# OpenResearchInstitute/ka9q-sdr

Measured on AMD Instinct MI355X. Metric: input Msamples/s + channels @ real-time, 16384-pt overlap-save, higher is better.
Workload: dtype f32

## Files before the change

### ka9q_sdr_amd/csrc/kq_bank.cpp

```cpp
#include <cstdarg>

#include "kq_bank.hpp"

using namespace kq::bank;

namespace {
thread_local std::string g_err;

int ilog2(unsigned v) {
  int l = 0;
  while ((1u << l) < v) l++;
  return l;
}
}

void kq_internal_set_error(const char *fmt, ...) {
  char buf[512];
  va_list ap;
  va_start(ap, fmt);
  vsnprintf(buf, sizeof buf, fmt, ap);
  va_end(ap);
  g_err = buf;
}

// ... 153 lines not shown
    b->fwd_mode = KQ_FWD_PRUNED;
  } else if (cfg->fwd_mode == KQ_FWD_FULL) {
    b->fwd_mode = KQ_FWD_FULL;
  } else {
    b->fwd_mode = (can_prune && g.Ndec != 256) ? KQ_FWD_PRUNED : KQ_FWD_FULL;
  }
  b->use64k = b->fwd_mode == KQ_FWD_FULL && can64k;
  if (b->fwd_mode == KQ_FWD_FULL && N > 16384 && !b->use64k && (!kq::split_supported(g) || cfg->compute_n0)) {
    kq_internal_set_error("N = %u: the full path beyond 16384 points needs N = 65536, or compute_n0 off and a split N = S x N1 with N1 <= 16384 a "
                          "size of its own (N = 32768; 19200, 24000, 38400, 48000 ...) and N/D small enough to sit beside it in LDS", N);
    return -1;
  }
  return 0;
}

static int create_alloc(kq_bank *b) {
  const kq_bank_config *cfg = &b->cfg;
  kq::Geom const &g = b->g;
  if (b->open_stream(cfg->stream)) return -1;
  size_t const C = cfg->max_channels, B = cfg->max_blocks;
  b->ring_cap = (size_t)(g.M - 1) + B * (size_t)g.L + (size_t)(g.L - 1);
  if (b->alloc(&b->ring[0], b->ring_cap, true)) return -1;
  if (b->alloc(&b->ring[1], b->ring_cap, true)) return -1;
  if (!(b->tw = kq::half_twiddles(g.tw_log2))) {
    kq_internal_set_error("kq_bank_create: no twiddle table of period 2^%d", g.tw_log2);
    return -1;
  }
  if (b->alloc(&b->chd.mode, C, true)) return -1;
  if (b->alloc(&b->chd.flags, C, true)) return -1;
  if (b->alloc(&b->chd.low, C, true)) return -1;
  if (b->alloc(&b->chd.high, C, true)) return -1;
  if (b->alloc(&b->chd.resp, C * g.Ndec, true)) return -1;
  if (b->alloc(&b->chd.aresp, C * (g.Ndec / 2 + 1), true)) return -1;
  if (b->alloc(&b->chd.fm_gain, C, true)) return -1;
  if (b->alloc(&b->chd.headroom, C, true)) return -1;
  if (b->alloc(&b->chd.recovery, C, true)) return -1;
  if (b->alloc(&b->chd.hangmax, C, true)) return -1;
  if (b->alloc(&b->chd.noise_gain, C, true)) return -1;
  if (b->alloc(&b->chd.hist_len, C, true)) return -1;
  if (b->alloc(&b->chd.hist2_len, C * kq::kOldLevels, true)) return -1;
  if (b->alloc(&b->chd.hist2_osc, 3 * C * kq::kOldLevels, true)) return -1;
  if (b->cfg.compute_n0 && (kq::full16k_supported(g) || b->use64k)) {
    size_t const nsub = b->use64k ? 4 : 1;
    if (b->alloc(&b->chd.n0lane, C * nsub * 256, true)) return -1;
    if (b->alloc(&b->chd.n0meta, C * nsub, true)) return -1;
    if (b->alloc(&b->chd.n0slot, C, true)) return -1;
  }
  if (b->use64k) {
    if (b->alloc(&b->big.sync, C * cfg->max_blocks * 12, true)) return -1;
    if (b->alloc(&b->big.n0part, C * cfg->max_blocks * 4, true)) return -1;
    if (b->alloc(&b->big.xs, C * cfg->max_blocks * (size_t)g.Ndec, true)) return -1;
    if (b->alloc_pinned(&b->big.err, 1)) return -1;
    *b->big.err = 0;
  }
  for (int k = 0; k < 2; k++)
    if (b->alloc(&b->osc_dev2[k], 8 * C + (B + sizeof(double) - 1) / sizeof(double) + (C * sizeof(int) + 7) / 8, true)) return -1;
  const char *ov = getenv("KQ_DEMOD_OVERLAP");
  b->overlap_mode = ov ? (atoi(ov) != 0 ? 1 : 0) : -1;
  bool const overlap = b->overlap_mode != 0;
  if (!overlap) b->stream2 = b->stream;
  if (overlap && b->new_stream(&b->stream2)) return -1;
  for (hipEvent_t &e : b->ev_demod_done)
    if (b->new_event(&e, hipEventDisableTiming)) return -1;
  b->stage_bytes = 8 * C * sizeof(double) + ((B + 7) & ~(size_t)7) + ((C * sizeof(int) + 7) & ~(size_t)7);
  b->patch_off = b->stage_bytes;
  b->stage_bytes += (size_t)kq_bank::kMaxPatch * kq_bank::kPatchBytes;
  b->bits_off = b->stage_bytes;
  b->stage_bytes += ((C + 63) / 64) * sizeof(unsigned long long);
  static_assert(kq_bank::kSlots == 4, "slot_bit_words");
  for (int k = 0; k < kq_bank::kSlots; k++) {
    if (b->alloc_pinned(&b->stage_host[k], b->stage_bytes) || b->new_event(&b->stage_ev[k], hipEventDefault) ||
        b->new_event(&b->stage_t0[k], hipEventDefault))
      return -1;
    memset(b->stage_host[k] + b->bits_off, 0, b->stage_bytes - b->bits_off);
  }
  if (b->alloc(&b->chd.fm_state, C, true)) return -1;
  if (b->alloc(&b->chd.lastaudio, C, true)) return -1;
  if (b->alloc(&b->chd.sq_count, C, true)) return -1;
  if (b->alloc(&b->chd.ahist, C * (size_t)(g.Mdec > 1 ? g.Mdec - 1 : 1), true)) return -1;
  if (!kq::demod64_supported(g)) {
    if (b->alloc(&b->fmout, C * B * (size_t)g.olen, true)) return -1;
    for (float *&h : b->fm_hist)
      if (b->alloc(&h, C * (size_t)(g.Mdec > 1 ? g.Mdec - 1 : 1), true)) return -1;
  }
  if (b->alloc(&b->chd.foffset, C, true)) return -1;
  if (b->alloc(&b->chd.pdev, C, true)) return -1;
  if (b->alloc(&b->chd.gain, C, true)) return -1;
  if (b->alloc(&b->chd.hang, C, true)) return -1;
  if (b->alloc(&b->chd.dc, C, true)) return -1;
  if (b->alloc(&b->chd.n0, C, true)) return -1;
  if (b->alloc(&b->chd.pl_ptr, C, true)) return -1;
  if (b->alloc(&b->chd.pl_last, C, true)) return -1;
  if (b->alloc(&b->chd.plfreq, C, true)) return -1;
  if (g.pl_n > 0) {
    if (b->alloc(&b->chd.plresp, (size_t)g.pl_n / 2 + 1, true)) return -1;
    if (b->alloc(&b->chd.plring, C * 16384, true)) return -1;
  }
  if (b->alloc(&b->pl.audio, C * B * 2 * (size_t)g.olen, true)) return -1;
  if (b->alloc(&b->pl.status, C * B, true)) return -1;
  for (int k = 0; k < 2; k++) {
    b->pl2[k].audio = b->pl.audio;
    b->pl2[k].status = b->pl.status;
    if (b->alloc(&b->pl2[k].filt, C * B * g.olen, true)) return -1;
    if (b->alloc(&b->pl2[k].n0raw, C * B, true)) return -1;
    if (b->alloc(&b->pl2[k].if_power, B * (1 + kq::kEnergySplitMax), true)) return -1;
    if (g.pl_n > 0 && b->alloc(&b->pl2[k].plout, C * B * g.pl_l, true)) return -1;
// ... 141 lines not shown
```

### ka9q_sdr_amd/csrc/kq_bank_call.cpp

```cpp
#include "kq_bank.hpp"

using namespace kq::bank;

namespace kq::bank {

void harvest_slot(kq_bank *b, int slot) {
  if (!b->stage_timed[slot]) return;
  b->stage_timed[slot] = false;
  float ms = 0;
  if (hipEventElapsedTime(&ms, b->stage_t0[slot], b->stage_ev[slot]) == hipSuccess && ms > 0) {
    b->acc.filter_ms += ms;
    if (ms > b->acc.filter_max_ms) {
      b->acc.filter_max_ms = ms;
      b->acc.filter_max_submit_ms = b->stage_submit_ms[slot];
      b->acc.filter_max_launch = b->stage_launch[slot];
    }
  } else
    (void)hipGetLastError();
}

void note_retune(kq_bank *b, int ch) {
  HostChan &h = b->chans[ch];
  int64_t const hist = (int64_t)b->g.M - 1;
  if (h.retuned && h.hist_old == hist) return;
// ... 330 lines not shown
      for (unsigned i = 0; i < k.nblocks; i++) {
        const float2 *X = k.spectrum + (size_t)i * g.N;
        size_t const cb = (size_t)c * g.max_blocks + i;
        if (b->cfg.compute_n0)
          kq::launch_n0_single(b->stream, X, g.N, g.samprate, b->chans[c].cfg.low, b->chans[c].cfg.high, k.pl.n0raw + cb);
        kq::launch_slave_bank(b->stream, X, k.chd.resp + (size_t)c * g.Ndec, k.pl.filt + cb * g.olen, g.N, g.Ndec, g.olen, isb ? 2 : 1,
                              b->tw, g.tw_log2);
      }
    }
  } else if (b->fwd_mode == KQ_FWD_PRUNED) {
    if (b->chan_tw_dirty) {
      kq::launch_pruned_tables(b->stream, g, k.chd, b->chan_tw, k.C);
      b->chan_tw_dirty = false;
    }
    if (kq::pruned_carries_iir(g)) iir_arm(b, k);
    kq::launch_filter_pruned(b->stream, g, k.chd, k.pl, k.window, b->chan_tw, act.n, nblocks, k.swept_pruned, act.list, b->big.iir);
    b->big.iir = kq::IirArgs{};
    if (k.nret > 0) {
      if (g.N > 16384)
        kq::launch_filter_split(b->stream, g, k.chd, k.pl, k.window, b->tw, k.nret, (int)k.nredo, k.retune_list);
      else
        full_launch(b, k, k.nret, (int)k.nredo, k.retune_list, 0, false);
    }
  } else if (b->use64k) {
    launch64k(b, k, act.n, nblocks, act.list, k.plain);
    if (k.plain && k.nret > 0) launch64k(b, k, k.nret, (int)k.nredo, k.retune_list, false);
  } else if (g.N > 16384) {
    kq::launch_filter_split(b->stream, g, k.chd, k.pl, k.window, b->tw, k.C, nblocks, nullptr);
  } else {
    int const steady_variant = k.swept_steady ? 2 : k.plain ? 1 : 0;
    if (k.mixed) {
      full_launch(b, k, (int)b->list_unswept_host.size(), nblocks, b->list_unswept_dev, 1);
      full_launch(b, k, (int)b->list_swept_host.size(), nblocks, b->list_swept_dev, steady_variant);
    } else {
      full_launch(b, k, act.n, nblocks, act.list, steady_variant);
    }
    if (k.use16k && (k.plain || k.mixed || k.swept_steady) && k.nret > 0)
      full_launch(b, k, k.nret, (int)k.nredo, k.retune_list, 0);
  }
}

int launch_energy_and_filter(kq_bank *b, Call &k) {
  kq::Geom const &g = b->g;
  int const slot = k.slot, pp = k.pp;
  if (ctl_flush(b, CTL_FILTER, b->stream)) return -1;
  {
    Scope t(b, 2, b->stream);
    kq::launch_block_energy_sum(b->stream, k.spectrum ? nullptr : k.window + (g.M - 1), g.L, k.spectrum ? 0 : (int)k.nblocks,
                                k.pl.if_power + b->cfg.max_blocks,
                                b->stage_host[slot], b->osc_dev2[pp],
                                k.nret ? k.ret_off + k.nret * sizeof(int) : 8 * k.Cmax * sizeof(double) + k.nblocks,
                                k.spectrum ? nullptr : k.paired, (int)(g.M - 1), k.steady ? b->osc_dev2[pp ^ 1] : nullptr, (unsigned)k.C,
                                (unsigned)k.Cmax, (double)(k.n_w - b->planes_n_w), (double)(b->out_abs - b->planes_out_abs),
                                b->stage_host[slot] + b->patch_off, k.npatch, b->stage_host[slot] + b->bits_off);
  }
  LAUNCH_CHECK("IF power");
  if (b->timing) {
    KQ_TRY(hipEventRecord(b->stage_t0[slot], b->stream));
    b->stage_timed[slot] = true;
    b->stage_h0[slot] = std::chrono::steady_clock::now();
    b->stage_launch[slot] = b->acc.filter_launches;
  }
  static bool const iir_in_filter_off = getenv("KQ_IIR_IN_FILTER") && atoi(getenv("KQ_IIR_IN_FILTER")) == 0;
  k.iir_off = iir_in_filter_off;
  launch_filter(b, k);
  LAUNCH_CHECK("pre-detection filter");
  b->acc.filter_launches++;
  b->acc.channel_blocks += (uint64_t)k.C * k.nblocks;
  KQ_TRY(hipEventRecord(b->stage_ev[slot], b->stream));
  if (b->timing) b->stage_submit_ms[slot] = std::chrono::duration<double, std::milli>(std::chrono::steady_clock::now() - b->stage_h0[slot]).count();
  return 0;
}

int launch_demodulators(kq_bank *b, Call &k) {
  kq::Geom const &g = b->g;
  int const pp = k.pp, nblocks = (int)k.nblocks;
  kq::Planes const &pl = k.pl;
  kq::ChanDev const &chd = k.chd;
  bool const agc_channels = !b->list_host[1].empty() || !b->list_host[2].empty();
  bool const overlap = b->stream2 != b->stream &&
                       (b->overlap_mode == 1 || (b->overlap_mode < 0 && !b->use64k && (b->pulled_since_call || agc_channels)));
  b->pulled_since_call = false;
  hipStream_t const ds = overlap ? b->stream2 : b->stream;
  int const prev = pp ^ 1;
  if (overlap)
    KQ_TRY(hipStreamWaitEvent(ds, b->stage_ev[k.slot], 0));
  else if (b->calls > 0 && b->demod_overlapped[prev])
    KQ_TRY(hipStreamWaitEvent(ds, b->ev_demod_done[prev], 0));
  if (b->out_pending) {
    KQ_TRY(hipStreamWaitEvent(ds, b->pull_done[(b->pulls - 1) % kq_bank::kPullRing], 0));
    b->out_pending = false;
  }
  if (ctl_flush(b, CTL_DEMOD, ds)) return -1;
  if (k.spectrum)
    KQ_TRY(hipMemsetAsync(pl.if_power, 0, k.nblocks * sizeof(float), ds));
  else if (!k.iir_done)
    kq::launch_block_energy_iir(ds, pl.if_power + b->cfg.max_blocks, g.L, nblocks,
                                reinterpret_cast<const unsigned char *>(b->osc_dev2[pp] + 8 * k.Cmax), b->energy_state, pl.if_power);
  {
    Scope t(b, 1, ds);
    int const nfm = (int)b->list_host[0].size(), nam = (int)b->list_host[1].size(), nlin = (int)b->list_host[2].size();
    bool const fused_fm = kq::demod64_supported(g);
    kq::launch_demod64(ds, g, chd, pl, b->list_dev[0], fused_fm ? nfm : 0, b->list_dev[1], nam, b->list_dev[2], nlin, nblocks,
                       b->cfg.compute_n0);
    if (!fused_fm) {
      kq::launch_demod_fm(ds, g, chd, pl, b->tw, b->list_dev[0], nfm, nblocks, b->cfg.compute_n0, b->fmout,
                          b->fm_hist[b->fm_hist_cur], b->fm_hist[b->fm_hist_cur ^ 1]);
// ... 166 lines not shown
```

### ka9q_sdr_amd/csrc/kq_device.hpp

```cpp
#pragma once
#include "kq_energy.hpp"
#include <hip/hip_runtime.h>
#include <stdint.h>

#include <functional>

#include "../../include/ka9q_hip.h"

struct filter_in;

namespace kq {

enum { FLAG_FLAT = 1, FLAG_ISB = 2, FLAG_STEREO = 4, FLAG_SQUARE = 8 };

struct PllState {
  double c_phase, c_freq;
  double f_phase, f_freq;
  float integrator, delta_f, snr, foffset, cphase;
  int lock_count, pll_lock, fft_samples, fft_ptr;
};

struct FftDim {
  int n;
  int log2n;
  int nf;
  unsigned char f[12];
  const unsigned short *rev;
  const float2 *twc;
  int tw_n;
};
FftDim fft_dim(int n, bool *ok);
bool fft_size_ok(int n);
const float2 *half_twiddles(int log2T);
enum { TABLE_HALF_TWIDDLES, TABLE_DIM_REV, TABLE_DIM_TW, TABLE_FULL16K };
const void *upload_once(int table, int size, size_t bytes, const std::function<void(void *)> &fill);

constexpr int kPllChunk = 64;
struct PllChunk {
  PllState *state;
  float2 *rings;
  float2 *side;
};

struct Geom {
  int N, L, M, D;
  FftDim dN, dNdec, dPl;
  int Ndec, olen, Mdec;
  int log2N, log2Ndec;
  int samprate;
  int tw_log2;
  int max_blocks;
  float dsamprate;
  int pl_n, pl_l;
};

constexpr int kOldLevels = 4;

struct ChanDev {
  int *mode;
  int *flags;
  int *fflags;
  float *low, *high;
  float2 *resp;
  float2 *aresp;
  float *fm_gain;
  float *headroom;
  float *recovery;
  int *hangmax;
  float *noise_gain;
  unsigned long long *n0lane;
  unsigned *n0meta;
  int *n0slot;
  double *lo_phase, *lo_freq, *lo_rate;
  double *hist_phase, *hist_freq, *hist_rate;
  int *hist_len;
  int *hist2_len;
  double *hist2_osc;
  double *sh_phase, *sh_freq;
  float2 *fm_state;
  float *lastaudio;
  int *sq_count;
  float *ahist;
  float *foffset, *pdev;
  float *gain;
  int *hang;
  float *dc;
  float *n0;
  float2 *plresp;
  float *plring;
  int *pl_ptr, *pl_last;
  float *plfreq;
};

struct Planes {
  float2 *filt;
  float *audio;
  kq_chan_status *status;
  float *n0raw;
  float *if_power;
  float *plout;
};

struct DeviceScope {
  int prev = -1;
  bool switched = false;
  explicit DeviceScope(int device) {
    if (device < 0) return;
    if (hipGetDevice(&prev) == hipSuccess && prev != device) switched = hipSetDevice(device) == hipSuccess;
  }
  ~DeviceScope() {
    if (switched) (void)hipSetDevice(prev);
  }
  DeviceScope(const DeviceScope &) = delete;
  DeviceScope &operator=(const DeviceScope &) = delete;
};

void ensure_dynamic_lds(const void *kernel, size_t bytes);

void launch_copy_to_host(hipStream_t s, const float *audio, float *haudio, int row, const kq_chan_status *status, void *hstatus,
                         size_t rows);
void launch_copy_pcm_to_host(hipStream_t s, const float *audio, short *hpcm, unsigned *hmask, int row,
                             const kq_chan_status *status, void *hstatus, size_t rows, const int *mode_compact = nullptr,
                             int max_blocks = 1);
void launch_ingest(hipStream_t s, const void *src, int format, float2 *dst, size_t nsamples, float scale);
constexpr int kEnergySplitMax = 16;
int block_energy_split(int L);
void launch_block_energy_sum(hipStream_t s, const float2 *newsamples, int L, int nblocks, float *sums, const void *params_host,
                             void *params_dev, size_t params_bytes, float2 *paired, int hist, const double *prev_planes = nullptr,
                             unsigned nchan = 0, unsigned cmax = 0, double adv = 0, double adv_out = 0, const void *patch_records_host = nullptr,
                             int npatch = 0, const void *patch_bits_host = nullptr);
void launch_ctl_apply(hipStream_t s, const void *queue_host, int nrec);
void launch_block_energy_iir(hipStream_t s, const float *sums, int L, int nblocks, const unsigned char *update, float *energy_state,
                             float *if_power);
void launch_pcm(hipStream_t s, const Geom &g, const Planes &pl, short *pcm, unsigned *mask, int nchan, int nblocks,
                const int *chan_list);
void launch_filter_full(hipStream_t s, const Geom &g, const ChanDev &ch, const Planes &pl, const float2 *window,
                        const float2 *tw, int nchan, int nblocks, int compute_n0, float2 *spec_dump, int spec_ch,
                        const int *chan_list);
bool split_supported(const Geom &g);
void launch_filter_split(hipStream_t s, const Geom &g, const ChanDev &ch, const Planes &pl, const float2 *window,
                         const float2 *tw, int nchan, int nblocks, const int *chan_list);
struct Big64 {
  unsigned long long *sync;
  float2 *n0part;
  float2 *xs;
  int *err;
  unsigned epoch;
  IirArgs iir;
};
bool full16k_supported(const Geom &g);
constexpr int kFull16kHalf = 16;
constexpr int full16k_bin(int t) { return (t >> 5) + 32 * (t & 31); }
void launch_filter_full16k(hipStream_t s, const Geom &g, const ChanDev &ch, const Planes &pl, const float2 *window,
                           const float2 *tw, int nchan, int nblocks, int compute_n0, float2 *spec_dump, int spec_ch,
                           const int *chan_list, int plain, const float2 *window_paired, const Big64 &big);
bool full16k_paired_supported(const Geom &g);
bool full64k_supported(const Geom &g);
void launch_filter_full64k(hipStream_t s, const Geom &g, const ChanDev &ch, const Planes &pl, const float2 *window,
                           const float2 *tw, int nchan, int nblocks, int compute_n0, float2 *spec_dump, int spec_ch,
                           const int *chan_list, bool plain, bool swept, const float2 *window_paired, const Big64 &big);
double full16k_sweep_limit();
double full64k_sweep_limit();
bool pruned_supported(const Geom &g);
void launch_filter_pruned(hipStream_t s, const Geom &g, const ChanDev &ch, const Planes &pl, const float2 *window,
                          const float2 *chan_tw, int nchan, int nblocks, bool swept, const int *chan_list, const IirArgs &iir = IirArgs{});
bool pruned_carries_iir(const Geom &g);
void launch_pruned_tables(hipStream_t s, const Geom &g, const ChanDev &ch, float2 *chan_tw, int nchan);
size_t pruned_table_elems(const Geom &g);
size_t demod_fm_lds_bytes(const Geom &g);
void launch_demod_fm(hipStream_t s, const Geom &g, const ChanDev &ch, const Planes &pl, const float2 *tw, const int *list_fm,
                     int n_fm, int nblocks, int compute_n0, float *fmout, const float *fm_hist_in, float *fm_hist_out);
void launch_pl_track(hipStream_t s, const Geom &g, const ChanDev &ch, const Planes &pl, const float2 *tw, const int *list_fm,
                     int n_fm, int nblocks);
bool demod64_supported(const Geom &g);
void launch_demod64(hipStream_t s, const Geom &g, const ChanDev &ch, const Planes &pl, const int *list_fm, int n_fm,
                    const int *list_am, int n_am, const int *list_lin, int n_lin, int nblocks, int compute_n0);
void launch_demod_pll(hipStream_t s, const Geom &g, const ChanDev &ch, const Planes &pl, const float2 *tw, const int *list_pll,
                      int n_pll, const PllChunk *chunks, const int *slot_of, int nblocks, int compute_n0);
void launch_fft_single(hipStream_t s, const float2 *in, float2 *out, const FftDim &d, int sign, const float2 *tw, int tw_log2);
int launch_fft_large(hipStream_t s, const float2 *in, float2 *out, float2 *tmp, int N, int sign, const float2 *tw, int tw_log2);
void launch_n0_single(hipStream_t s, const float2 *fdomain, int N, int samprate, float low, float high, float *out);
void launch_slave_single(hipStream_t s, const float2 *fdomain, const float2 *resp, float2 *out, int N, int Ndec,
                         int in_real, int out_type, const float2 *tw, int tw_log2);
// ... 10 lines not shown
```

### ka9q_sdr_amd/csrc/kq_full16k.hip

```cpp
#include "kq_device.hpp"
#include "kq_ldsfft.hpp"
#include <cmath>
#include <type_traits>

#include "kq_lane.hpp"
#include "kq_regfft.hpp"

#ifdef KQ_TIMELINE
__device__ unsigned long long kq_timeline[64][8][12];
#define KQ_STAMP(i)                                                                        \
  do {                                                                                     \
    __builtin_amdgcn_sched_barrier(0);                                                     \
    if (blockIdx.y == (gridDim.y > 40 ? 40 : gridDim.y / 2) && (blockIdx.x & 15) == 0 && (blockIdx.x >> 4) < 64 &&      \
        (threadIdx.x & 63) == 0)                                                           \
      kq_timeline[blockIdx.x >> 4][threadIdx.x >> 6][i] = clock64();                       \
    __builtin_amdgcn_sched_barrier(0);                                                     \
  } while (0)
extern "C" int kq_debug_timeline(unsigned long long *dst) {
  return hipMemcpyFromSymbol(dst, HIP_SYMBOL(kq_timeline), sizeof(kq_timeline)) == hipSuccess ? 0 : -1;
}
#else
#define KQ_STAMP(i)
#endif

// ... 76 lines not shown
    for (;;) {
      w = __hip_atomic_load(slots + t, __ATOMIC_RELAXED, __HIP_MEMORY_SCOPE_AGENT);
      if ((unsigned)(w >> 32) == tag || ++it > (1 << 18)) break;
      __builtin_amdgcn_s_sleep(8);
    }
    if ((unsigned)(w >> 32) != tag) {
      *err = 1;
      w = 0x7fc00000u;
    }
    out[t] = __uint_as_float((unsigned)w);
  }
  __syncthreads();
}

}

template <bool N0, bool DUMP, int PLAIN, bool PAIRED, int BIG, int EPI>
__global__ __launch_bounds__(kT, 4) void k_filter_full16k(Geom g, ChanDev ch, Planes pl, const float2 *__restrict__ window,
                                                       const float2 *__restrict__ tw, const float2 *__restrict__ tab,
                                                       float2 *__restrict__ spec_dump, int spec_ch,
                                                       const int *__restrict__ chan_list, Big64 big) {
  extern __shared__ __attribute__((aligned(16))) float2 xch[];
  __shared__ __attribute__((aligned(16))) float2 stab[(kT / 64) * (BIG ? 128 : 32)];
  __shared__ float sib_f[BIG ? 12 : 1];
  constexpr int kNfull = BIG ? 4 * kN : kN;
  int const r4 = BIG ? (int)(blockIdx.x & 3) : 0;
  __shared__ __attribute__((aligned(16))) float2 tw2[16 * kTw2Pitch];
  __shared__ float red_f[2][kT / 64];
  __shared__ float red_c[kT / 64];
  __shared__ int red_i[2][kT / 64];
  int const t = threadIdx.x;
  int const Ndec = g.Ndec;
  KQ_STAMP(0);
  __builtin_amdgcn_s_setprio(3);
  v2f v[32];
  rsrc_t const xr = make_rsrc(window + (size_t)blockIdx.y * g.L, kNfull * (unsigned)sizeof(float2));
  unsigned const toff = (unsigned)t * (unsigned)sizeof(float2);
  auto load_rows = [&](int first, int last) {
    if constexpr (PAIRED) {
#pragma unroll
      for (int n1 = first; n1 < last; n1 += 2)
        buf_ld4(v[rfft::bitrev5(n1)], v[rfft::bitrev5(n1 + 1)], xr, 2 * toff, (unsigned)(n1 / 2) * (unsigned)(1024 * sizeof(float2)));
    } else {
#pragma unroll
      for (int n1 = first; n1 < last; n1++) v[rfft::bitrev5(n1)] = buf_ld2(xr, toff, (unsigned)n1 * (unsigned)(512 * sizeof(float2)));
    }
  };
  auto load_window = [&]() { load_rows(0, 32); };
  rsrc_t const tabr = make_rsrc(tab, kTabSize * (unsigned)sizeof(float2));
  v2f tlo[3], thi[7];
  int const cidx = BIG ? (int)(blockIdx.x >> 2) : (int)blockIdx.x;
  int const c = chan_list ? chan_list[cidx] : cidx, b = blockIdx.y;
  v2f pt = (v2f){1.f, 0.f};
  if constexpr (BIG != 0) {
    double const ph0 = ch.lo_phase[c], f0 = ch.lo_freq[c], rs = ch.lo_rate[c];
    double const hp0 = ch.hist_phase[c], hf0 = ch.hist_freq[c], hr = ch.hist_rate[c];
    double const mbase = (double)b * g.L;
    int const n_old = (hp0 != ph0 || hf0 != f0 || hr != rs) ? ch.hist_len[c] - b * g.L : 0;
    bool const retuned = n_old > 0;
    if (PLAIN || (!retuned && fabs(rs) <= kSweepLimit64k)) {
      constexpr bool kSwept = !PLAIN || BIG == 2;
      v2f sa[2][4], sb[2][4];
      auto issue = [&](int i, int slot) {
#pragma unroll
        for (int j = 0; j < 4; j++) {
          if constexpr (PAIRED) {
            buf_ld4(sa[slot][j], sb[slot][j], xr, 2 * toff, (unsigned)(16 * j + i) * (unsigned)(1024 * sizeof(float2)));
          } else {
            sa[slot][j] = buf_ld2(xr, toff, (unsigned)(32 * j + 2 * i) * (unsigned)(512 * sizeof(float2)));
            sb[slot][j] = buf_ld2(xr, toff, (unsigned)(32 * j + 2 * i + 1) * (unsigned)(512 * sizeof(float2)));
          }
        }
      };
      issue(0, 0);
      issue(1, 1);
      __builtin_amdgcn_sched_barrier(0);
      float2 *const sw = stab + (t >> 6) * 128;
      {
        int const lane = t & 63;
        double const wv = (double)(64 * (t >> 6));
#pragma unroll
        for (int e2 = 0; e2 < 2; e2++) {
          int const e = lane + 64 * e2, j = e >> 5, n1 = e & 31;
          double const R = (double)(16384 * j + 512 * n1), U = mbase + R;
          double turns = f0 * U - (double)(r4 * n1) * (1.0 / 128.0) - 0.25 * (double)(r4 * j);
          if (kSwept) turns += rs * (0.5 * U * (U - 1.0) + R * wv);
          sw[e] = phasor_turns(turns);
        }
      }
      {
        double const td = (double)t;
        double turns = ph0 + f0 * td - (double)(r4 * t) * (1.0 / 65536.0);
        if (kSwept) turns += rs * (mbase * td + 0.5 * td * (td - 1.0));
        pt = phasor2(turns);
      }
      float const kbf = kSwept ? (float)(2.0 * M_PI * 16384.0 * rs * (double)(t & 63)) : 0.f;
      v2f const kb = (v2f){kbf, kbf};
      __builtin_amdgcn_fence(__ATOMIC_RELEASE, "wavefront");
      __builtin_amdgcn_wave_barrier();
      __builtin_amdgcn_fence(__ATOMIC_ACQUIRE, "wavefront");
      const float4 *const tp = reinterpret_cast<const float4 *>(sw);
#pragma unroll
      for (int i = 0; i < 16; i++) {
        int const slot = i & 1;
        float4 tt[4];
#pragma unroll
        for (int j = 0; j < 4; j++) tt[j] = tp[16 * j + i];
#pragma unroll
        for (int e = 0; e < 2; e++) {
          int const n1 = 2 * i + e;
          v2f x[4], w[4];
#pragma unroll
          for (int j = 0; j < 4; j++) {
            x[j] = e ? sb[slot][j] : sa[slot][j];
            w[j] = e ? (v2f){tt[j].z, tt[j].w} : (v2f){tt[j].x, tt[j].y};
          }
          v2f z;
          if constexpr (kSwept) {
            v2f const y0 = pk_cmul(x[0], w[0]), y1 = pk_cmul(x[1], w[1]), y2 = pk_cmul(x[2], w[2]), y3 = pk_cmul(x[3], w[3]);
            v2f const a = y1 + y3, bb = y2 + y3;
            v2f const S = (y0 + y2) + a;
            v2f const W = rfft::pk_fma(bb, (v2f){2.f, 2.f}, a);
            v2f const Uu = n1 ? rfft::pk_fma(S, (v2f){n1 / 32.f, n1 / 32.f}, W) : W;
            asm("v_pk_fma_f32 %0, %1, %2, %3 op_sel:[1,0,0] op_sel_hi:[0,1,1] neg_lo:[0,1,0]" : "=v"(z) : "v"(Uu), "v"(kb), "v"(S));
          } else {
            z = pk_cmul(x[0], w[0]);
            z = rfft::pk_cmadd(x[1], w[1], z);
            z = rfft::pk_cmadd(x[2], w[2], z);
            z = rfft::pk_cmadd(x[3], w[3], z);
          }
          v[rfft::bitrev5(n1)] = z;
        }
        if (i + 2 < 16) issue(i + 2, slot);
      }
    } else {
      OlderOsc older;
      load_older(ch, c, b * g.L, n_old > 0, older);
#pragma unroll
      for (int n1 = 0; n1 < 32; n1++) {
        v2f acc = (v2f){0.f, 0.f};
        for (int j = 0; j < 4; j++) {
          int const i = 16384 * j + 512 * n1 + t;
          double const m = mbase + i;
          bool const old = i < n_old;
          double pp = old ? hp0 : ph0, ff = old ? hf0 : f0, rr = old ? hr : rs;
          pick_older(older, i, pp, ff, rr);
          double turns = pp + ff * m;
          if (rr != 0.0) turns += rr * (0.5 * m * (m - 1.0));
          turns -= (double)(r4 * (512 * n1 + t)) * (1.0 / 65536.0) + 0.25 * (double)(r4 * j);
          acc = rfft::pk_cmadd(buf_ld2(xr, toff, (unsigned)(32 * j + n1) * (unsigned)(512 * sizeof(float2))), phasor2(turns), acc);
        }
        v[rfft::bitrev5(n1)] = acc;
      }
    }
  }
  if constexpr (PLAIN && BIG == 0) {
    double const ph0 = ch.lo_phase[c], f0 = ch.lo_freq[c];
    double const rs = PLAIN == 2 ? ch.lo_rate[c] : 0.0;
    load_rows(0, 12);
    __builtin_amdgcn_sched_barrier(0);
    float2 *const sw = stab + (t >> 6) * 32;
    if ((t & 63) < 32) {
      double const R = (double)(512 * (t & 63));
      double turns = f0 * R;
      if constexpr (PLAIN == 2) turns += rs * (0.5 * R * (R - 1.0) + R * ((double)b * g.L + (double)(t & ~63)));
      sw[t & 63] = phasor_turns(turns);
    }
    __builtin_amdgcn_sched_barrier(0);
    load_rows(12, 22);
    __builtin_amdgcn_sched_barrier(0);
    {
      double const A = (double)b * g.L + t;
      double turns = ph0 + f0 * A;
      if constexpr (PLAIN == 2) turns += rs * (0.5 * A * (A - 1.0));
      pt = phasor2(turns);
    }
    __builtin_amdgcn_sched_barrier(0);
    load_rows(22, 32);
  }
  twiddle32_fetch(tlo, thi, tabr, t);
  v2f const tw2_mine = buf_ld2(tabr, toff, (unsigned)kTabTw2 * 8u);
  KQ_STAMP(10);

  if constexpr (BIG == 0) {
    double const ph0 = ch.lo_phase[c], f0 = ch.lo_freq[c], r = ch.lo_rate[c];
    double const hp0 = ch.hist_phase[c], hf0 = ch.hist_freq[c], hr = ch.hist_rate[c];
    double const mbase = (double)b * g.L;
    int const n_old = (hp0 != ph0 || hf0 != f0 || hr != r) ? ch.hist_len[c] - b * g.L : 0;
    bool const retuned = n_old > 0;
    if (PLAIN || (r == 0.0 && !retuned)) {
      float2 *const sw = stab + (t >> 6) * 32;
      if constexpr (!PLAIN) {
        load_window();
        if ((t & 63) < 32) sw[t & 63] = phasor_turns(f0 * (double)(512 * (t & 63)));
        pt = phasor2(ph0 + f0 * (mbase + t));
      }
      KQ_STAMP(11);
      __builtin_amdgcn_fence(__ATOMIC_RELEASE, "wavefront");
      __builtin_amdgcn_wave_barrier();
      __builtin_amdgcn_fence(__ATOMIC_ACQUIRE, "wavefront");
      if constexpr (PLAIN == 2) {
        float const kbf = (float)(2.0 * M_PI * 512.0 * r * (double)(t & 63));
        v2f const kb = (v2f){kbf, kbf};
        v2f th = (v2f){0.f, 0.f};
#pragma unroll
        for (int n1 = 1; n1 < 32; n1++) {
          v2f const y = pk_cmul(v[rfft::bitrev5(n1)], ld2(sw + n1));
          th = th + kb;
          v2f z;
          asm("v_pk_fma_f32 %0, %1, %2, %3 op_sel:[1,0,0] op_sel_hi:[0,1,1] neg_lo:[0,1,0]" : "=v"(z) : "v"(y), "v"(th), "v"(y));
          v[rfft::bitrev5(n1)] = z;
        }
      } else {
#pragma unroll
        for (int n1 = 1; n1 < 32; n1++) v[rfft::bitrev5(n1)] = pk_cmul(v[rfft::bitrev5(n1)], ld2(sw + n1));
      }
    } else if constexpr (!PLAIN) {
      OlderOsc older;
      load_older(ch, c, b * g.L, n_old > 0, older);
#pragma unroll
      for (int n1 = 0; n1 < 32; n1++) {
        int const i = 512 * n1 + t;
        double const m = mbase + i;
        bool const old = i < n_old;
        double pp = old ? hp0 : ph0, ff = old ? hf0 : f0, rr = old ? hr : r;
        pick_older(older, i, pp, ff, rr);
        double turns = pp + ff * m;
        if (rr != 0.0) turns += rr * (0.5 * m * (m - 1.0));
        v[rfft::bitrev5(n1)] = pk_cmul(buf_ld2(xr, toff, (unsigned)n1 * (unsigned)(512 * sizeof(float2))), phasor2(turns));
      }
    }
  }

  KQ_STAMP(1);
  __builtin_amdgcn_s_setprio(0);
  rfft::fft_dit_pk<32>(v);
  twiddle32(v, tlo, thi, pt);

  KQ_STAMP(2);
  v2f u[32];
  tw2[(t >> 5) * kTw2Pitch + (t & 31)] = make_float2(tw2_mine.x, tw2_mine.y);
#if defined(KQ_ABLATE) && (KQ_ABLATE & 1)
#pragma unroll
  for (int n2 = 0; n2 < 32; n2++) u[n2] = v[n2];
#else
  {
    int const rd = ((t >> 4) & 15) * kRow1 + (t & 15);
#pragma unroll
// ... 420 lines not shown
      G[bitrev((unsigned)k, g.log2Ndec)] = gn;
    }
    G[bitrev((unsigned)p, g.log2Ndec)] = gp;
  }
  lds_fft<+1>(G, g.log2Ndec, tw, g.tw_log2);
  float2 *o = pl.filt + cb * g.olen;
  for (int i = t; i < g.olen; i += blockDim.x) o[i] = G[Ndec - g.olen + i];
}

bool full16k_supported(const Geom &g) {
  return g.N == kN && 2 * g.Ndec <= kXchElems && g.Ndec >= 4;
}

static const float2 *twiddle_tables() {
  return (const float2 *)upload_once(TABLE_FULL16K, kN, kTabSize * sizeof(float2), [](void *bytes) {
    float2 *h = (float2 *)bytes;
    auto w = [](long long e) {
      double const ang = -2.0 * M_PI * (double)(e % kN) / kN;
      return make_float2((float)cos(ang), (float)sin(ang));
    };
    for (int t = 0; t < kT; t++)
      for (int e = 0; e < 10; e++)
        h[kTabP1 + 2 * (kT * (e >> 1) + t) + (e & 1)] = e < 3 ? w((long long)(e + 1) * t) : w(4LL * (e - 2) * t);
    for (int n3 = 0; n3 < 16; n3++)
      for (int k2 = 0; k2 < 32; k2++) h[kTabTw2 + 32 * n3 + k2] = w(32LL * n3 * k2);
    for (int st = 1; st <= 5; st++)
      for (int t = 0; t < 64; t++) {
        int const half = 1 << st;
        double const ang = M_PI * (double)(t & (half - 1)) / half;
        h[kTabEpi + (st - 1) * 64 + t] = (t & half) ? make_float2((float)cos(ang), (float)sin(ang)) : make_float2(1.f, 0.f);
      }
  });
}

bool full16k_paired_supported(const Geom &g) {
  return (full16k_supported(g) || full64k_supported(g)) && g.L % 1024 == 0 && (g.M - 1) % 1024 == 0;
}

bool full64k_supported(const Geom &g) { return g.N == 4 * kN && g.Ndec >= 4 && g.Ndec <= 16384; }
double full64k_sweep_limit() { return kSweepLimit64k; }
double full16k_sweep_limit() { return kSweepLimit16k; }

void launch_filter_full16k(hipStream_t s, const Geom &g, const ChanDev &ch, const Planes &pl, const float2 *window,
                           const float2 *tw, int nchan, int nblocks, int compute_n0, float2 *spec_dump, int spec_ch,
                           const int *chan_list, int plain, const float2 *window_paired, const Big64 &big) {
  size_t const lds_bytes = (size_t)kXchElems * sizeof(float2);
  const float2 *tab = twiddle_tables();
  if (!tab) {
    launch_filter_full(s, g, ch, pl, window, tw, nchan, nblocks, compute_n0, spec_dump, spec_ch, chan_list);
    if (big.iir.sums)
      launch_block_energy_iir(s, big.iir.sums, big.iir.L, big.iir.nblocks, big.iir.update, big.iir.state, big.iir.if_power);
    return;
  }
  bool const n0 = compute_n0 && ch.n0lane && ch.n0meta;
  bool const dump = spec_dump != nullptr;
  bool const paired = plain && window_paired != nullptr;
  auto go = [&](auto kernel) {
    ensure_dynamic_lds((const void *)kernel, lds_bytes);
    hipLaunchKernelGGL(kernel, dim3(nchan, nblocks), dim3(kT), lds_bytes, s, g, ch, pl, paired ? window_paired : window, tw, tab,
                       spec_dump, spec_ch, chan_list, big);
  };
  int const epi = dump ? 0 : g.Ndec == 64 ? 1 : (g.Ndec >= 128 && g.Ndec <= 512) ? 2 : 0;
  auto pick3 = [&](auto n0c, auto dumpc, auto epic) {
    constexpr bool kN0 = decltype(n0c)::value, kDump = decltype(dumpc)::value;
    constexpr int kEpi = decltype(epic)::value;
    if (plain == 2)
      paired ? go(k_filter_full16k<kN0, kDump, 2, true, 0, kEpi>) : go(k_filter_full16k<kN0, kDump, 2, false, 0, kEpi>);
    else if (paired)
      go(k_filter_full16k<kN0, kDump, 1, true, 0, kEpi>);
    else
      plain ? go(k_filter_full16k<kN0, kDump, 1, false, 0, kEpi>) : go(k_filter_full16k<kN0, kDump, 0, false, 0, kEpi>);
  };
  auto pick = [&](auto n0c, auto dumpc) {
    if constexpr (decltype(dumpc)::value) {
      pick3(n0c, dumpc, std::integral_constant<int, 0>{});
    } else {
      if (epi == 1)
        pick3(n0c, dumpc, std::integral_constant<int, 1>{});
      else if (epi == 2)
        pick3(n0c, dumpc, std::integral_constant<int, 2>{});
      else
        pick3(n0c, dumpc, std::integral_constant<int, 0>{});
    }
  };
  using T = std::true_type;
  using F = std::false_type;
  if (n0)
    dump ? pick(T{}, T{}) : pick(T{}, F{});
  else
    dump ? pick(F{}, T{}) : pick(F{}, F{});
}

void launch_filter_full64k(hipStream_t s, const Geom &g, const ChanDev &ch, const Planes &pl, const float2 *window,
                           const float2 *tw, int nchan, int nblocks, int compute_n0, float2 *spec_dump, int spec_ch,
                           const int *chan_list, bool plain, bool swept, const float2 *window_paired, const Big64 &big) {
  size_t const lds_bytes = (size_t)kXchElems * sizeof(float2);
  const float2 *tab = twiddle_tables();
  if (!tab) {
    if (big.iir.sums)
      launch_block_energy_iir(s, big.iir.sums, big.iir.L, big.iir.nblocks, big.iir.update, big.iir.state, big.iir.if_power);
    return;
  }
  bool const n0 = compute_n0 && ch.n0lane && ch.n0meta;
  bool const dump = spec_dump != nullptr;
  bool const paired = plain && window_paired != nullptr;
  auto go = [&](auto kernel) {
// ... 27 lines not shown
```

### ka9q_sdr_amd/csrc/kq_kernels.hip

```cpp
#include <algorithm>
#include <map>
#include <mutex>
#include <utility>

#include "kq_device.hpp"
#include "kq_ctl.hpp"
#include "kq_energy.hpp"
#include "kq_ldsfft.hpp"

namespace kq {

void ensure_dynamic_lds(const void *kernel, size_t bytes) {
  static std::mutex mu;
  static std::map<std::pair<const void *, int>, size_t> limit;
  int dev = 0;
  if (hipGetDevice(&dev) != hipSuccess) return;
  std::lock_guard<std::mutex> lock(mu);
  size_t &cur = limit[{kernel, dev}];
  if (bytes > cur) {
    (void)hipFuncSetAttribute(kernel, hipFuncAttributeMaxDynamicSharedMemorySize, (int)bytes);
    cur = bytes;
  }
}

__global__ void k_ingest(const void *__restrict__ src, int format, float2 *__restrict__ dst, size_t n, float gain) {
  size_t const stride = (size_t)gridDim.x * blockDim.x;
  for (size_t i = (size_t)blockIdx.x * blockDim.x + threadIdx.x; i < n; i += stride) {
    float2 v;
    if (format == KQ_IQ_S16) {
      short2 const q = reinterpret_cast<const short2 *>(src)[i];
      float const sc = 1.f / 32767.f;
      v = make_float2(q.x * sc, q.y * sc);
    } else if (format == KQ_IQ_S8) {
      char2 const q = reinterpret_cast<const char2 *>(src)[i];
      float const sc = 1.f / 127.f;
      v = make_float2(q.x * sc, q.y * sc);
    } else {
      v = reinterpret_cast<const float2 *>(src)[i];
    }
    dst[i] = make_float2(v.x * gain, v.y * gain);
  }
}

void launch_ingest(hipStream_t s, const void *src, int format, float2 *dst, size_t nsamples, float gain) {
  if (nsamples == 0) return;
  int const threads = 256;
  size_t blocks = (nsamples + threads - 1) / threads;
  if (blocks > 2048) blocks = 2048;
  hipLaunchKernelGGL(k_ingest, dim3((unsigned)blocks), dim3(threads), 0, s, src, format, dst, nsamples, gain);
}

__device__ __forceinline__ double frac_turns(double ph, double f, double n) {
  double const hi = f * n, lo = __fma_rn(f, n, -hi);
  double const p = ph + ((hi - floor(hi)) + lo);
  return p - floor(p);
}
__global__ void k_block_energy_sum(const float2 *__restrict__ x, int L, float *__restrict__ sums, int nblocks, int split,
                                   const unsigned long long *__restrict__ params_host,
                                   unsigned long long *__restrict__ params_dev, unsigned nwords, int copy_wgs,
                                   float2 *__restrict__ paired, int hist, const double *__restrict__ prev, unsigned nchan,
                                   unsigned cmax, double adv, double adv_out, int hist_wgs,
                                   const unsigned long long *__restrict__ patch_rec, int npatch,
                                   const unsigned long long *__restrict__ patch_bits) {
  int const pcol = 2 * (threadIdx.x & 511) + (threadIdx.x >> 9);
  int const nsum = nblocks * split;
  if ((int)blockIdx.x >= nsum + copy_wgs + hist_wgs) {
    int const j = ((int)blockIdx.x - nsum - copy_wgs - hist_wgs) * (int)blockDim.x + (int)threadIdx.x;
    if (j >= npatch) return;
    const unsigned long long *r = patch_rec + (size_t)j * 9;
    unsigned const c = (unsigned)r[0];
    if (c >= cmax) return;
    double *planes = reinterpret_cast<double *>(params_dev);
#pragma unroll
    for (int k = 0; k < 8; k++) planes[(size_t)k * cmax + c] = __longlong_as_double((long long)r[1 + k]);
    return;
  }
  if ((int)blockIdx.x >= nsum + copy_wgs) {
    int const base = ((int)blockIdx.x - nsum - copy_wgs) * 8192;
    for (int j = 0; j < 8 && base + 1024 * j < hist; j++) paired[base + 1024 * j + pcol] = (x - hist)[base + 1024 * j + threadIdx.x];
    return;
  }
  if ((int)blockIdx.x >= nsum) {
    unsigned const i = (blockIdx.x - nsum) * blockDim.x + threadIdx.x;
    if (!prev) {
      if (i < nwords) params_dev[i] = params_host[i];
      return;
    }
    if (i < nchan) {
      if (patch_bits && ((patch_bits[i >> 6] >> (i & 63)) & 1ull)) return;
      double *out = reinterpret_cast<double *>(params_dev);
      double const ph = prev[i], f = prev[cmax + i], r = prev[2 * (size_t)cmax + i];
      double const sp = prev[3 * (size_t)cmax + i], sf = prev[4 * (size_t)cmax + i];
      double p = frac_turns(ph, f, adv);
      if (r != 0.0) {
        p += r * (0.5 * adv * (adv - 1.0));
        p -= floor(p);
      }
      double const f2 = f + r * adv;
      out[i] = p;
      out[cmax + i] = f2;
      out[2 * (size_t)cmax + i] = r;
      out[3 * (size_t)cmax + i] = frac_turns(sp, sf, adv_out);
      out[4 * (size_t)cmax + i] = sf;
      out[5 * (size_t)cmax + i] = p;
      out[6 * (size_t)cmax + i] = f2;
      out[7 * (size_t)cmax + i] = r;
    } else if (i - nchan < nwords - 8 * cmax) {
      params_dev[8 * (size_t)cmax + (i - nchan)] = params_host[8 * (size_t)cmax + (i - nchan)];
    }
    return;
  }
  __shared__ float red_f[16];
  __shared__ int red_i[16];
  int const blk = (int)blockIdx.x / split, part = (int)blockIdx.x % split;
  const float2 *p = x + (size_t)blk * L;
  float acc = 0;
  int dummy = 0;
  int const first = part * (int)blockDim.x + (int)threadIdx.x, stride = split * (int)blockDim.x;
  float2 *o = paired ? paired + hist + (size_t)blk * L : nullptr;
  for (int i0 = first; i0 < L; i0 += 4 * stride) {
    float2 v[4];
#pragma unroll
    for (int j = 0; j < 4; j++) v[j] = i0 + j * stride < L ? p[i0 + j * stride] : make_float2(0.f, 0.f);
#pragma unroll
    for (int j = 0; j < 4; j++) {
      int const i = i0 + j * stride;
      if (i < L) {
        acc += cnrm(v[j]);
        if (o) o[(i - (int)threadIdx.x) + pcol] = v[j];
      }
    }
  }
  block_sum_fi(acc, dummy, red_f, red_i);
  if (threadIdx.x == 0) sums[blockIdx.x] = acc;
}
__global__ void k_block_energy_iir(const float *__restrict__ sums, int split, const unsigned char *__restrict__ update,
                                   int nblocks, int L, float *__restrict__ state, float *__restrict__ if_power) {
  block_energy_iir_wave(sums, split, update, nblocks, L, state, if_power, (int)threadIdx.x);
}

int block_energy_split(int L) {
  int const trips = (L + 1023) / 1024;
  return std::max(1, std::min(kEnergySplitMax, (trips + 2) / 3));
}

void launch_block_energy_sum(hipStream_t s, const float2 *newsamples, int L, int nblocks, float *sums, const void *params_host,
                             void *params_dev, size_t params_bytes, float2 *paired, int hist, const double *prev_planes,
                             unsigned nchan, unsigned cmax, double adv, double adv_out, const void *patch_records_host, int npatch,
                             const void *patch_bits_host) {
  unsigned const nwords = (unsigned)((params_bytes + 7) / 8);
  unsigned const work = prev_planes ? nchan + (nwords - 8 * cmax) : nwords;
  int const copy_wgs = (int)((work + 1023) / 1024);
  int const hist_wgs = paired ? (hist + 8191) / 8192 : 0;
  int const split = block_energy_split(L);
  if (!prev_planes || !patch_records_host || !patch_bits_host) npatch = 0;
  int const patch_wgs = (npatch + 1023) / 1024;
  hipLaunchKernelGGL(k_block_energy_sum, dim3(nblocks * split + copy_wgs + hist_wgs + patch_wgs), dim3(1024), 0, s, newsamples, L, sums,
                     nblocks, split, static_cast<const unsigned long long *>(params_host),
                     static_cast<unsigned long long *>(params_dev), nwords, copy_wgs, paired, hist, prev_planes, nchan, cmax, adv,
                     adv_out, hist_wgs, static_cast<const unsigned long long *>(patch_records_host), npatch,
                     npatch ? static_cast<const unsigned long long *>(patch_bits_host) : nullptr);
}

__global__ void __launch_bounds__(256) k_ctl_apply(const unsigned char *__restrict__ q) { ctl_apply_record(q, blockIdx.x, threadIdx.x, 256); }
void launch_ctl_apply(hipStream_t s, const void *queue_host, int nrec) {
  if (nrec > 0) hipLaunchKernelGGL(k_ctl_apply, dim3(nrec), dim3(256), 0, s, static_cast<const unsigned char *>(queue_host));
}

void launch_block_energy_iir(hipStream_t s, const float *sums, int L, int nblocks, const unsigned char *update, float *energy_state,
                             float *if_power) {
  hipLaunchKernelGGL(k_block_energy_iir, dim3(1), dim3(64), 0, s, sums, block_energy_split(L), update, nblocks, L, energy_state,
                     if_power);
}

typedef unsigned int u32x4 __attribute__((ext_vector_type(4)));
__global__ void __launch_bounds__(256) k_copy_to_host(const float *__restrict__ audio, float *__restrict__ haudio, int row,
                                                      const kq_chan_status *__restrict__ status, u32x4 *__restrict__ hstatus,
                                                      size_t rows, size_t status16) {
  size_t const stride = (size_t)gridDim.x * blockDim.x;
  size_t const tid = (size_t)blockIdx.x * blockDim.x + threadIdx.x;
  if (haudio) {
    int const sub = (int)(tid & 15);
    for (size_t r = tid >> 4; r < rows; r += stride >> 4) {
      int const n = min(status[r].nout, row);
      const float *src = audio + r * row;
      float *dst = haudio + r * row;
      for (int i = 4 * sub; i < n; i += 64) {
        u32x4 const v = *reinterpret_cast<const u32x4 *>(src + i);
        __builtin_nontemporal_store(v, reinterpret_cast<u32x4 *>(dst + i));
      }
    }
  }
  const u32x4 *sp = reinterpret_cast<const u32x4 *>(status);
  if (hstatus)
    for (size_t i = tid; i < status16; i += stride) __builtin_nontemporal_store(sp[i], hstatus + i);
}
void launch_copy_to_host(hipStream_t s, const float *audio, float *haudio, int row, const kq_chan_status *status, void *hstatus,
                         size_t rows) {
  size_t const bytes = rows * ((haudio ? (size_t)row * sizeof(float) : 0) + (hstatus ? sizeof(kq_chan_status) : 0));
  unsigned const wgs = (unsigned)std::min<size_t>(64, std::max<size_t>(4, (bytes + (2u << 20) - 1) >> 21));
  hipLaunchKernelGGL(k_copy_to_host, dim3(wgs), dim3(256), 0, s, audio, haudio, row, status, (u32x4 *)hstatus, rows,
                     rows * sizeof(kq_chan_status) / 16);
}

template <bool COMPACT>
__global__ void __launch_bounds__(256) k_copy_pcm_to_host(const float *__restrict__ audio, short *__restrict__ hpcm,
                                                          unsigned *__restrict__ hmask, int row,
                                                          const kq_chan_status *__restrict__ status, u32x4 *__restrict__ hstatus,
                                                          size_t rows, size_t status16, const int *__restrict__ mode,
                                                          int max_blocks) {
  size_t const stride = (size_t)gridDim.x * blockDim.x;
  size_t const tid = (size_t)blockIdx.x * blockDim.x + threadIdx.x;
  int const sub = (int)(tid & 15);
  for (size_t r = tid >> 4; r < rows; r += stride >> 4) {
// ... 103 lines not shown
```

Measured before the change: 376,900.

## Cache per-channel fixed-frequency oscillator phasor tables instead of recomputing in filter

For fixed-frequency (non-swept) channels, the filter kernel's double-precision phasor computation is replaced with lookups into per-channel tables: row steps, lane steps, wave steps and per-block phasors, plus a per-call starting phase. The tables are rebuilt only when the channel frequency changes, tracked by a frequency tag, inside extra workgroups of the energy/param-copy kernel. The per-call start phasor is refreshed in the param copy paths. This removes fp64 sincos work from the hot filter kernel, at the cost of extra memory, more launch complexity, float product rounding error, and the risk of stale tables.

```diff
diff --git a/ka9q_sdr_amd/csrc/kq_bank.cpp b/ka9q_sdr_amd/csrc/kq_bank.cpp
--- a/ka9q_sdr_amd/csrc/kq_bank.cpp
+++ b/ka9q_sdr_amd/csrc/kq_bank.cpp
@@ -229,6 +229,12 @@
     if (b->alloc(&b->big.xs, C * cfg->max_blocks * (size_t)g.Ndec, true)) return -1;
     if (b->alloc_pinned(&b->big.err, 1)) return -1;
     *b->big.err = 0;
+  }
+  if (kq::full16k_supported(g) && b->fwd_mode != KQ_FWD_PRUNED) {
+    if (b->alloc(&b->chd.osc_tab, C * (kq::kOscFixed + B), true)) return -1;
+    if (b->alloc(&b->chd.osc_pc, C, true)) return -1;
+    if (b->alloc(&b->chd.osc_tag, C)) return -1;
+    KQ_TRY(hipMemsetAsync(b->chd.osc_tag, 0xff, C * sizeof(unsigned long long), b->stream));
   }
   for (int k = 0; k < 2; k++)
     if (b->alloc(&b->osc_dev2[k], 8 * C + (B + sizeof(double) - 1) / sizeof(double) + (C * sizeof(int) + 7) / 8, true)) return -1;
diff --git a/ka9q_sdr_amd/csrc/kq_bank_call.cpp b/ka9q_sdr_amd/csrc/kq_bank_call.cpp
--- a/ka9q_sdr_amd/csrc/kq_bank_call.cpp
+++ b/ka9q_sdr_amd/csrc/kq_bank_call.cpp
@@ -406,7 +406,8 @@
                                 k.nret ? k.ret_off + k.nret * sizeof(int) : 8 * k.Cmax * sizeof(double) + k.nblocks,
                                 k.spectrum ? nullptr : k.paired, (int)(g.M - 1), k.steady ? b->osc_dev2[pp ^ 1] : nullptr, (unsigned)k.C,
                                 (unsigned)k.Cmax, (double)(k.n_w - b->planes_n_w), (double)(b->out_abs - b->planes_out_abs),
-                                b->stage_host[slot] + b->patch_off, k.npatch, b->stage_host[slot] + b->bits_off);
+                                b->stage_host[slot] + b->patch_off, k.npatch, b->stage_host[slot] + b->bits_off,
+                                kq::OscTabs{b->chd.osc_tab, b->chd.osc_tag, b->chd.osc_pc, (int)b->cfg.max_blocks});
   }
   LAUNCH_CHECK("IF power");
   if (b->timing) {
diff --git a/ka9q_sdr_amd/csrc/kq_device.hpp b/ka9q_sdr_amd/csrc/kq_device.hpp
--- a/ka9q_sdr_amd/csrc/kq_device.hpp
+++ b/ka9q_sdr_amd/csrc/kq_device.hpp
@@ -55,6 +55,8 @@
 };
 
 constexpr int kOldLevels = 4;
+constexpr int kOscRow = 0, kOscLane = 32, kOscWave = 96, kOscFixed = 104;
+constexpr unsigned long long kOscNoTag = ~0ull;
 
 struct ChanDev {
   int *mode;
@@ -72,6 +74,9 @@
   unsigned *n0meta;
   int *n0slot;
   double *lo_phase, *lo_freq, *lo_rate;
+  float2 *osc_tab;
+  unsigned long long *osc_tag;
+  float2 *osc_pc;
   double *hist_phase, *hist_freq, *hist_rate;
   int *hist_len;
   int *hist2_len;
@@ -124,11 +129,17 @@
                              int max_blocks = 1);
 void launch_ingest(hipStream_t s, const void *src, int format, float2 *dst, size_t nsamples, float scale);
 constexpr int kEnergySplitMax = 16;
+struct OscTabs {
+  float2 *tab = nullptr;
+  unsigned long long *tag = nullptr;
+  float2 *pc = nullptr;
+  int max_blocks = 0;
+};
 int block_energy_split(int L);
 void launch_block_energy_sum(hipStream_t s, const float2 *newsamples, int L, int nblocks, float *sums, const void *params_host,
                              void *params_dev, size_t params_bytes, float2 *paired, int hist, const double *prev_planes = nullptr,
                              unsigned nchan = 0, unsigned cmax = 0, double adv = 0, double adv_out = 0, const void *patch_records_host = nullptr,
-                             int npatch = 0, const void *patch_bits_host = nullptr);
+                             int npatch = 0, const void *patch_bits_host = nullptr, const OscTabs &osc = OscTabs{});
 void launch_ctl_apply(hipStream_t s, const void *queue_host, int nrec);
 void launch_block_energy_iir(hipStream_t s, const float *sums, int L, int nblocks, const unsigned char *update, float *energy_state,
                              float *if_power);
diff --git a/ka9q_sdr_amd/csrc/kq_full16k.hip b/ka9q_sdr_amd/csrc/kq_full16k.hip
--- a/ka9q_sdr_amd/csrc/kq_full16k.hip
+++ b/ka9q_sdr_amd/csrc/kq_full16k.hip
@@ -152,6 +152,8 @@
   int const cidx = BIG ? (int)(blockIdx.x >> 2) : (int)blockIdx.x;
   int const c = chan_list ? chan_list[cidx] : cidx, b = blockIdx.y;
   v2f pt = (v2f){1.f, 0.f};
+  v2f osc_s = pt, osc_l = pt;
+  v2f osc_pc = pt, osc_rb = pt, osc_qw = pt;
   if constexpr (BIG != 0) {
     double const ph0 = ch.lo_phase[c], f0 = ch.lo_freq[c], rs = ch.lo_rate[c];
     double const hp0 = ch.hist_phase[c], hf0 = ch.hist_freq[c], hr = ch.hist_rate[c];
@@ -255,28 +257,47 @@
     }
   }
   if constexpr (PLAIN && BIG == 0) {
-    double const ph0 = ch.lo_phase[c], f0 = ch.lo_freq[c];
-    double const rs = PLAIN == 2 ? ch.lo_rate[c] : 0.0;
-    load_rows(0, 12);
-    __builtin_amdgcn_sched_barrier(0);
-    float2 *const sw = stab + (t >> 6) * 32;
-    if ((t & 63) < 32) {
-      double const R = (double)(512 * (t & 63));
-      double turns = f0 * R;
-      if constexpr (PLAIN == 2) turns += rs * (0.5 * R * (R - 1.0) + R * ((double)b * g.L + (double)(t & ~63)));
-      sw[t & 63] = phasor_turns(turns);
-    }
-    __builtin_amdgcn_sched_barrier(0);
-    load_rows(12, 22);
-    __builtin_amdgcn_sched_barrier(0);
-    {
-      double const A = (double)b * g.L + t;
-      double turns = ph0 + f0 * A;
-      if constexpr (PLAIN == 2) turns += rs * (0.5 * A * (A - 1.0));
-      pt = phasor2(turns);
-    }
-    __builtin_amdgcn_sched_barrier(0);
-    load_rows(22, 32);
+    if constexpr (PLAIN == 1) {
+      typedef const v2f __attribute__((address_space(4))) *uniform_f2;
+      int const cu = __builtin_amdgcn_readfirstlane(c);
+      unsigned const rec_n = (unsigned)(kOscFixed + g.max_blocks);
+      const float2 *const rec = ch.osc_tab + (size_t)cu * rec_n;
+      osc_pc = *(uniform_f2)(ch.osc_pc + cu);
+      osc_rb = ((uniform_f2)rec)[kOscFixed + b];
+      osc_qw = ((uniform_f2)rec)[kOscWave + __builtin_amdgcn_readfirstlane(t >> 6)];
+      load_rows(0, 12);
+      __builtin_amdgcn_sched_barrier(0);
+      rsrc_t const oscr = make_rsrc(rec, rec_n * (unsigned)sizeof(float2));
+      osc_s = buf_ld2(oscr, (unsigned)(t & 31) * 8u, kOscRow * 8u);
+      osc_l = buf_ld2(oscr, (unsigned)(t & 63) * 8u, kOscLane * 8u);
+      __builtin_amdgcn_sched_barrier(0);
+      load_rows(12, 22);
+      __builtin_amdgcn_sched_barrier(0);
+      load_rows(22, 32);
+    } else {
+      double const ph0 = ch.lo_phase[c], f0 = ch.lo_freq[c];
+      double const rs = PLAIN == 2 ? ch.lo_rate[c] : 0.0;
+      load_rows(0, 12);
+      __builtin_amdgcn_sched_barrier(0);
+      float2 *const sw = stab + (t >> 6) * 32;
+      if ((t & 63) < 32) {
+        double const R = (double)(512 * (t & 63));
+        double turns = f0 * R;
+        if constexpr (PLAIN == 2) turns += rs * (0.5 * R * (R - 1.0) + R * ((double)b * g.L + (double)(t & ~63)));
+        sw[t & 63] = phasor_turns(turns);
+      }
+      __builtin_amdgcn_sched_barrier(0);
+      load_rows(12, 22);
+      __builtin_amdgcn_sched_barrier(0);
+      {
+        double const A = (double)b * g.L + t;
+        double turns = ph0 + f0 * A;
+        if constexpr (PLAIN == 2) turns += rs * (0.5 * A * (A - 1.0));
+        pt = phasor2(turns);
+      }
+      __builtin_amdgcn_sched_barrier(0);
+      load_rows(22, 32);
+    }
   }
   twiddle32_fetch(tlo, thi, tabr, t);
   v2f const tw2_mine = buf_ld2(tabr, toff, (unsigned)kTabTw2 * 8u);
@@ -294,6 +315,10 @@
         load_window();
         if ((t & 63) < 32) sw[t & 63] = phasor_turns(f0 * (double)(512 * (t & 63)));
         pt = phasor2(ph0 + f0 * (mbase + t));
+      }
+      if constexpr (PLAIN == 1) {
+        if ((t & 63) < 32) sw[t & 63] = make_float2(osc_s.x, osc_s.y);
+        pt = pk_cmul(pk_cmul(osc_pc, osc_rb), pk_cmul(osc_qw, osc_l));
       }
       KQ_STAMP(11);
       __builtin_amdgcn_fence(__ATOMIC_RELEASE, "wavefront");
@@ -820,6 +845,7 @@
       launch_block_energy_iir(s, big.iir.sums, big.iir.L, big.iir.nblocks, big.iir.update, big.iir.state, big.iir.if_power);
     return;
   }
+  if (plain == 1 && !ch.osc_tab) plain = 0;
   bool const n0 = compute_n0 && ch.n0lane && ch.n0meta;
   bool const dump = spec_dump != nullptr;
   bool const paired = plain && window_paired != nullptr;
diff --git a/ka9q_sdr_amd/csrc/kq_kernels.hip b/ka9q_sdr_amd/csrc/kq_kernels.hip
--- a/ka9q_sdr_amd/csrc/kq_kernels.hip
+++ b/ka9q_sdr_amd/csrc/kq_kernels.hip
@@ -61,9 +61,55 @@
                                    float2 *__restrict__ paired, int hist, const double *__restrict__ prev, unsigned nchan,
                                    unsigned cmax, double adv, double adv_out, int hist_wgs,
                                    const unsigned long long *__restrict__ patch_rec, int npatch,
-                                   const unsigned long long *__restrict__ patch_bits) {
+                                   const unsigned long long *__restrict__ patch_bits, int patch_wgs, OscTabs osc) {
   int const pcol = 2 * (threadIdx.x & 511) + (threadIdx.x >> 9);
   int const nsum = nblocks * split;
+  if ((int)blockIdx.x >= nsum + copy_wgs + hist_wgs + patch_wgs) {
+    __shared__ unsigned osc_c[4];
+    __shared__ unsigned long long osc_f[4];
+    int const q = (int)threadIdx.x >> 8, e0 = (int)threadIdx.x & 255;
+    int const j = ((int)blockIdx.x - nsum - copy_wgs - hist_wgs - patch_wgs) * 4 + q;
+    if (e0 == 0) {
+      unsigned long long f = kOscNoTag, r = 0;
+      unsigned c = cmax;
+      if (prev) {
+        if (j < npatch) {
+          c = (unsigned)patch_rec[(size_t)j * 9];
+          f = patch_rec[(size_t)j * 9 + 2];
+          r = patch_rec[(size_t)j * 9 + 3];
+        }
+      } else if ((unsigned)j < nchan) {
+        c = (unsigned)j;
+        f = params_host[cmax + c];
+        r = params_host[2 * (size_t)cmax + c];
+      }
+      unsigned long long build = kOscNoTag;
+      if (c < cmax) {
+        bool const fixed = __longlong_as_double((long long)r) == 0.0;
+        if (!fixed)
+          osc.tag[c] = kOscNoTag;
+        else if (osc.tag[c] != f) {
+          osc.tag[c] = f;
+          build = f;
+        }
+      }
+      osc_f[q] = build;
+      osc_c[q] = c;
+    }
+    __syncthreads();
+    if (osc_f[q] == kOscNoTag) return;
+    double const f0 = __longlong_as_double((long long)osc_f[q]);
+    int const n = kOscFixed + osc.max_blocks;
+    float2 *const rec = osc.tab + (size_t)osc_c[q] * n;
+    for (int e = e0; e < n; e += 256) {
+      double const k = e < kOscLane ? (double)(512 * e)
+                       : e < kOscWave ? (double)(e - kOscLane)
+                       : e < kOscFixed ? (double)(64 * (e - kOscWave))
+                                       : (double)(e - kOscFixed) * (double)L;
+      rec[e] = phasor_turns(f0 * k);
+    }
+    return;
+  }
   if ((int)blockIdx.x >= nsum + copy_wgs + hist_wgs) {
     int const j = ((int)blockIdx.x - nsum - copy_wgs - hist_wgs) * (int)blockDim.x + (int)threadIdx.x;
     if (j >= npatch) return;
@@ -73,6 +119,7 @@
     double *planes = reinterpret_cast<double *>(params_dev);
 #pragma unroll
     for (int k = 0; k < 8; k++) planes[(size_t)k * cmax + c] = __longlong_as_double((long long)r[1 + k]);
+    if (osc.tab) osc.pc[c] = phasor_turns(__longlong_as_double((long long)r[1]));
     return;
   }
   if ((int)blockIdx.x >= nsum + copy_wgs) {
@@ -83,7 +130,11 @@
   if ((int)blockIdx.x >= nsum) {
     unsigned const i = (blockIdx.x - nsum) * blockDim.x + threadIdx.x;
     if (!prev) {
-      if (i < nwords) params_dev[i] = params_host[i];
+      if (i < nwords) {
+        unsigned long long const w = params_host[i];
+        params_dev[i] = w;
+        if (osc.tab && i < nchan && i < cmax) osc.pc[i] = phasor_turns(__longlong_as_double((long long)w));
+      }
       return;
     }
     if (i < nchan) {
@@ -105,6 +156,10 @@
       out[5 * (size_t)cmax + i] = p;
       out[6 * (size_t)cmax + i] = f2;
       out[7 * (size_t)cmax + i] = r;
+      if (osc.tab) {
+        osc.pc[i] = phasor_turns(p);
+        if (r != 0.0) osc.tag[i] = kOscNoTag;
+      }
     } else if (i - nchan < nwords - 8 * cmax) {
       params_dev[8 * (size_t)cmax + (i - nchan)] = params_host[8 * (size_t)cmax + (i - nchan)];
     }
@@ -147,7 +202,7 @@
 void launch_block_energy_sum(hipStream_t s, const float2 *newsamples, int L, int nblocks, float *sums, const void *params_host,
                              void *params_dev, size_t params_bytes, float2 *paired, int hist, const double *prev_planes,
                              unsigned nchan, unsigned cmax, double adv, double adv_out, const void *patch_records_host, int npatch,
-                             const void *patch_bits_host) {
+                             const void *patch_bits_host, const OscTabs &osc) {
   unsigned const nwords = (unsigned)((params_bytes + 7) / 8);
   unsigned const work = prev_planes ? nchan + (nwords - 8 * cmax) : nwords;
   int const copy_wgs = (int)((work + 1023) / 1024);
@@ -155,11 +210,12 @@
   int const split = block_energy_split(L);
   if (!prev_planes || !patch_records_host || !patch_bits_host) npatch = 0;
   int const patch_wgs = (npatch + 1023) / 1024;
-  hipLaunchKernelGGL(k_block_energy_sum, dim3(nblocks * split + copy_wgs + hist_wgs + patch_wgs), dim3(1024), 0, s, newsamples, L, sums,
+  int const osc_wgs = osc.tab ? (int)(((prev_planes ? (unsigned)npatch : nchan) + 3) / 4) : 0;
+  hipLaunchKernelGGL(k_block_energy_sum, dim3(nblocks * split + copy_wgs + hist_wgs + patch_wgs + osc_wgs), dim3(1024), 0, s, newsamples, L, sums,
                      nblocks, split, static_cast<const unsigned long long *>(params_host),
                      static_cast<unsigned long long *>(params_dev), nwords, copy_wgs, paired, hist, prev_planes, nchan, cmax, adv,
                      adv_out, hist_wgs, static_cast<const unsigned long long *>(patch_records_host), npatch,
-                     npatch ? static_cast<const unsigned long long *>(patch_bits_host) : nullptr);
+                     npatch ? static_cast<const unsigned long long *>(patch_bits_host) : nullptr, patch_wgs, osc);
 }
 
 __global__ void __launch_bounds__(256) k_ctl_apply(const unsigned char *__restrict__ q) { ctl_apply_record(q, blockIdx.x, threadIdx.x, 256); }
```

New measurement: 380,600 (median of 6 runs). No clear change (+1.0%).
